# josehu07/summerset

Hardware: NVIDIA B200
Metric: RS shard GB/s on the fused RSPaxos accept step (RS(3,2) encode + quorum tally); consensus slots committed/s in slots_committed_per_s (higher is better)
Workload: dtype u8

## Files before the change

summerset_b200/csrc/horner_row_kernels.cuh:

```cuda
#pragma once
#include "device_common.cuh"
#include "static_codes.hpp"

namespace ssb {

using dev::funnel16;
using dev::keep_bytes;
using dev::msb_mask;

#ifndef SS_KMAXP
#define SS_KMAXP 8
#endif

struct EncRowGen {
    const uint8_t *data;
    uint64_t data_stride;
    uint8_t *plane[16];
    uint64_t shard_stride;
    uint32_t emit_data;
    dev::FlagWait wait;
    uint32_t n, len, L, vpc, fast_cols;
    uint32_t d, p;
    uint32_t pack_m, tail_ctas, ntail;
    const uint32_t *hmT8;
    uint8_t top[SS_KMAXP];
    const uint64_t *planes;
    uint32_t R, threshold;
    uint64_t *committed;
    uint32_t *commit_bar;
};

__device__ __forceinline__ uint32_t xtime_word(uint32_t x) { return ((x * 2u) & 0xfefefefeu) ^ (msb_mask(x) & 0x1d1d1d1du); }

template <int D, bool MASKED, bool EXACT>
__device__ __forceinline__ int row_load_column(const EncRowGen &P, const uint8_t *__restrict__ src, uint32_t k, uint4 (&x)[D]) {
    auto clamp16 = [](int64_t r) { return r > 16 ? 16 : (r < 0 ? 0 : static_cast<int>(r)); };
    const int d = EXACT ? D : static_cast<int>(P.d);
    uint4 lo[D], hi[D];
#pragma unroll
    for (int i = 0; i < D; ++i) {
        lo[i] = make_uint4(0u, 0u, 0u, 0u);
        hi[i] = lo[i];
        if (i < d) {
            const uint32_t pos = static_cast<uint32_t>(i) * P.L + k;
            const uint32_t s = (static_cast<uint32_t>(i) * P.L) & 15u;
            const int nv = MASKED ? clamp16(static_cast<int64_t>(P.len) - pos) : 16;
            if (!MASKED || nv > 0) lo[i] = dev::ldg128(src + pos - s);
            if (s != 0u && (!MASKED || static_cast<int>(s) + nv > 16)) hi[i] = dev::ldg128(src + pos - s + 16u);
        }
    }
    const int onv = MASKED ? clamp16(static_cast<int64_t>(P.L) - k) : 16;
#pragma unroll
    for (int i = 0; i < D; ++i) {
        x[i] = lo[i];
        if (i < d) {
            const uint32_t s = (static_cast<uint32_t>(i) * P.L) & 15u;
            if (s != 0u) x[i] = funnel16(lo[i], hi[i], s);
            if (MASKED) {
                const int nv = clamp16(static_cast<int64_t>(P.len) - (static_cast<uint32_t>(i) * P.L + k));
                x[i] = keep_bytes(x[i], nv < onv ? nv : onv);
            }
        }
    }
    return onv;
}

template <int CODE, int J, int D>
__device__ __forceinline__ uint4 static_parity_row(const uint4 (&x)[D]) {
    static_assert(D == static_code_d(CODE), "static code width");
    constexpr int top = static_code_top(CODE, J);
    uint4 acc = make_uint4(0u, 0u, 0u, 0u);
#pragma unroll
    for (int kk = 7; kk >= 0; --kk) {
        if (kk > top) continue;
        if (kk != top) {
            acc.x = xtime_word(acc.x); acc.y = xtime_word(acc.y);
            acc.z = xtime_word(acc.z); acc.w = xtime_word(acc.w);
        }
#pragma unroll
        for (int i = 0; i < D; ++i)
            if ((static_code_coef(CODE, J, i) >> kk) & 1u) {
                acc.x ^= x[i].x; acc.y ^= x[i].y; acc.z ^= x[i].z; acc.w ^= x[i].w;
            }
    }
    return acc;
}

template <int D, int CODE, bool MASKED>
__device__ __forceinline__ void parity_rows(const EncRowGen &P, const uint4 (&x)[D], int onv, uint64_t out_off) {
    if (P.emit_data) {
#pragma unroll
        for (int i = 0; i < D; ++i)
            if (CODE != kCodeGeneric || static_cast<uint32_t>(i) < P.d) dev::stg128_cs(P.plane[i] + out_off, x[i]);
    }
    if constexpr (CODE != kCodeGeneric) {
        static_assert(D == static_code_d(CODE), "static code width");
#pragma unroll
        for (int j = 0; j < static_code_p(CODE); ++j) {
            const int top = static_code_top(CODE, j);
            uint4 acc = make_uint4(0u, 0u, 0u, 0u);
#pragma unroll
            for (int kk = 7; kk >= 0; --kk) {
                if (kk > top) continue;
                if (kk != top) {
                    acc.x = xtime_word(acc.x); acc.y = xtime_word(acc.y);
                    acc.z = xtime_word(acc.z); acc.w = xtime_word(acc.w);
                }
#pragma unroll
                for (int i = 0; i < D; ++i)
                    if ((static_code_coef(CODE, j, i) >> kk) & 1u) {
                        acc.x ^= x[i].x; acc.y ^= x[i].y; acc.z ^= x[i].z; acc.w ^= x[i].w;
                    }
            }
            if (MASKED) acc = keep_bytes(acc, onv);
            dev::stg128_cs(P.plane[D + j] + out_off, acc);
        }
    } else {
        for (uint32_t j = 0; j < P.p; ++j) {
            const uint4 *hm = reinterpret_cast<const uint4 *>(P.hmT8 + j * 64u);
            uint4 acc = make_uint4(0u, 0u, 0u, 0u);
            const int top = P.top[j];
            for (int kk = top; kk >= 0; --kk) {
                const uint4 m0 = __ldg(hm + kk * 2);
                const uint4 m1 = D > 4 ? __ldg(hm + kk * 2 + 1) : make_uint4(0u, 0u, 0u, 0u);
                const uint32_t mk[8] = {m0.x, m0.y, m0.z, m0.w, m1.x, m1.y, m1.z, m1.w};
                if (kk != top) {
                    acc.x = xtime_word(acc.x); acc.y = xtime_word(acc.y);
                    acc.z = xtime_word(acc.z); acc.w = xtime_word(acc.w);
                }
#pragma unroll
                for (int i = 0; i < D; ++i) {
                    acc.x ^= x[i].x & mk[i];
                    acc.y ^= x[i].y & mk[i];
                    acc.z ^= x[i].z & mk[i];
                    acc.w ^= x[i].w & mk[i];
                }
            }
            if (MASKED) acc = keep_bytes(acc, onv);
            dev::stg128_cs(P.plane[P.d + j] + out_off, acc);
        }
    }
}

template <int D, int CODE, bool MASKED>
__device__ __forceinline__ void horner_row_column(const EncRowGen &P, const uint8_t *__restrict__ src, uint64_t out_off, uint32_t k) {
    uint4 x[D];
    const int onv = row_load_column<D, MASKED, CODE != kCodeGeneric>(P, src, k, x);
    parity_rows<D, CODE, MASKED>(P, x, onv, out_off + k);
}

template <int D, bool ALIGNED>
struct RawColumn {
    uint4 lo[D];
    uint4 hi[ALIGNED ? 1 : D];
};
template <int D, bool ALIGNED, bool EXACT>
__device__ __forceinline__ void raw_issue(const EncRowGen &P, const uint8_t *__restrict__ src, uint32_t k, RawColumn<D, ALIGNED> &r) {
    const int d = EXACT ? D : static_cast<int>(P.d);
#pragma unroll
    for (int i = 0; i < D; ++i) {
        if (i < d) {
            const uint32_t pos = static_cast<uint32_t>(i) * P.L + k;
            const uint32_t s = ALIGNED ? 0u : (static_cast<uint32_t>(i) * P.L) & 15u;
            r.lo[i] = dev::ldg128(src + pos - s);
            if constexpr (!ALIGNED) {
                if (i > 0) {
                    r.hi[i] = make_uint4(0u, 0u, 0u, 0u);
                    if (s != 0u) r.hi[i] = dev::ldg128(src + pos - s + 16u);
                }
            }
        } else {
            r.lo[i] = make_uint4(0u, 0u, 0u, 0u);
        }
    }
}
template <int D, bool ALIGNED, bool EXACT>
__device__ __forceinline__ void raw_finish(const EncRowGen &P, const RawColumn<D, ALIGNED> &r, uint4 (&x)[D]) {
    const int d = EXACT ? D : static_cast<int>(P.d);
#pragma unroll
    for (int i = 0; i < D; ++i) {
        x[i] = r.lo[i];
        if constexpr (!ALIGNED) {
            if (i > 0 && i < d) {
                const uint32_t s = (static_cast<uint32_t>(i) * P.L) & 15u;
                if (s != 0u) x[i] = funnel16(r.lo[i], r.hi[i], s);
            }
        }
    }
}

template <int D, int CODE, int MAXT, int MINB>
__global__ void __launch_bounds__(MAXT, MINB) horner_encode_row_kernel(const __grid_constant__ EncRowGen P) {
    const uint32_t lane = threadIdx.x & 31u, wid = threadIdx.x >> 5, nblk = blockDim.x >> 5;
    if (P.emit_data) dev::cta_wait_flags(P.wait);
    if (P.planes != nullptr) {
        const uint32_t per = (P.n + gridDim.x - 1) / gridDim.x;
        const uint32_t lo = blockIdx.x * per;
        const uint32_t hi = lo + per < P.n ? lo + per : P.n;
        for (uint32_t g = lo + threadIdx.x; g < hi; g += blockDim.x) {
            const uint64_t w = dev::tally_word(P.planes, P.R, P.n, g, P.threshold);
            P.committed[g] = w;
            if (P.commit_bar != nullptr) P.commit_bar[g] = dev::commit_prefix(w);
        }
    }
    uint32_t wb = wid;
#pragma unroll 1
    for (uint32_t g = blockIdx.x; g < P.n; g += gridDim.x) {
        const uint8_t *src = P.data + static_cast<uint64_t>(g) * P.data_stride;
        const uint64_t out_off = static_cast<uint64_t>(g) * P.shard_stride;
        for (uint32_t vb = 0; vb < P.vpc; vb += blockDim.x) {
            const uint32_t v = vb + wb * 32u + lane;
            const bool masked = vb + wb * 32u + 32u > P.fast_cols;
            if (v >= P.vpc) continue;
            if (!masked) horner_row_column<D, CODE, false>(P, src, out_off, v * 16u);
            else horner_row_column<D, CODE, true>(P, src, out_off, v * 16u);
        }
        wb = (wb + 1u == nblk) ? 0u : wb + 1u;
    }
}

template <int D, bool ALIGNED, bool PIPE>
SSB_HD constexpr int packed_min_blocks() {
    if (!PIPE) return D <= 3 ? 6 : D <= 5 ? 5 : D <= 6 ? 4 : 3;
    constexpr int need = 4 * D + (ALIGNED ? 4 * D : 8 * D - 4) + 22;
    constexpr int b = 65536 / (256 * need);
    return b > 6 ? 6 : (b < 1 ? 1 : b);
}

template <int D, int CODE, bool ALIGNED, bool PIPE>
__global__ void __launch_bounds__(256, packed_min_blocks<D, ALIGNED, PIPE>()) horner_encode_packed_kernel(const __grid_constant__ EncRowGen P) {
    if (P.emit_data) dev::cta_wait_flags(P.wait);
    if (P.planes != nullptr) {
        const uint32_t per = (P.n + gridDim.x - 1) / gridDim.x;
        const uint32_t lo = blockIdx.x * per;
        const uint32_t hi = lo + per < P.n ? lo + per : P.n;
        for (uint32_t g = lo + threadIdx.x; g < hi; g += blockDim.x) {
            const uint64_t w = dev::tally_word(P.planes, P.R, P.n, g, P.threshold);
            P.committed[g] = w;
            if (P.commit_bar != nullptr) P.commit_bar[g] = dev::commit_prefix(w);
        }
    }
    if (blockIdx.x < P.tail_ctas) {
        const uint64_t item = static_cast<uint64_t>(blockIdx.x) * blockDim.x + threadIdx.x;
        const uint64_t g = P.ntail == 1u ? item : item / P.ntail;
        if (g >= P.n) return;
        const uint32_t col = P.fast_cols + static_cast<uint32_t>(item - g * P.ntail);
        horner_row_column<D, CODE, true>(P, P.data + g * P.data_stride, g * P.shard_stride, col * 16u);
        return;
    }
    const uint32_t cg = threadIdx.x / P.fast_cols;
    const uint32_t k = (threadIdx.x - cg * P.fast_cols) * 16u;
    if (cg >= P.pack_m) return;
    const uint64_t step = static_cast<uint64_t>(gridDim.x - P.tail_ctas) * P.pack_m;
    uint64_t g = static_cast<uint64_t>(blockIdx.x - P.tail_ctas) * P.pack_m + cg;
    if (g >= P.n) return;
    if constexpr (!PIPE) {
#pragma unroll 1
        for (; g < P.n; g += step)
            horner_row_column<D, CODE, false>(P, P.data + g * P.data_stride, g * P.shard_stride, k);
        return;
    }
    RawColumn<D, ALIGNED> raw;
    raw_issue<D, ALIGNED, CODE != kCodeGeneric>(P, P.data + g * P.data_stride, k, raw);
#pragma unroll 1
    while (true) {
        uint4 x[D];
        raw_finish<D, ALIGNED, CODE != kCodeGeneric>(P, raw, x);
        const uint64_t gn = g + step;
        if (gn < P.n) raw_issue<D, ALIGNED, CODE != kCodeGeneric>(P, P.data + gn * P.data_stride, k, raw);
        parity_rows<D, CODE, false>(P, x, 16, g * P.shard_stride + k);
        if (gn >= P.n) break;
        g = gn;
    }
}


}
```

summerset_b200/csrc/jit.cu:

```cuda
#include <dlfcn.h>
#include <nvrtc.h>

#include <cstdio>
#include <cstring>
#include <mutex>
#include <string>
#include <vector>

#include "gf256.hpp"
#include "ss_internal.hpp"
#include "static_codes.hpp"

namespace ssb {

static const char *kJitSource =
#include "jit_source.inc"
    ;

struct NvrtcApi {
    void *handle = nullptr;
    nvrtcResult (*CreateProgram)(nvrtcProgram *, const char *, const char *, int, const char *const *, const char *const *) = nullptr;
    nvrtcResult (*DestroyProgram)(nvrtcProgram *) = nullptr;
    nvrtcResult (*CompileProgram)(nvrtcProgram, int, const char *const *) = nullptr;
    nvrtcResult (*AddNameExpression)(nvrtcProgram, const char *) = nullptr;
    nvrtcResult (*GetLoweredName)(nvrtcProgram, const char *, const char **) = nullptr;
    nvrtcResult (*GetCUBINSize)(nvrtcProgram, size_t *) = nullptr;
    nvrtcResult (*GetCUBIN)(nvrtcProgram, char *) = nullptr;
    nvrtcResult (*GetProgramLogSize)(nvrtcProgram, size_t *) = nullptr;
    nvrtcResult (*GetProgramLog)(nvrtcProgram, char *) = nullptr;
    const char *(*GetErrorString)(nvrtcResult) = nullptr;
    bool ok = false;
};

static NvrtcApi &nvrtc_api() {
    static NvrtcApi api;
    static std::once_flag once;
    std::call_once(once, [] {
        const char *names[] = {"libnvrtc.so.12", "libnvrtc.so", "/usr/local/cuda/lib64/libnvrtc.so.12", "/usr/local/cuda/lib64/libnvrtc.so"};
        for (const char *n : names) {
            api.handle = dlopen(n, RTLD_NOW | RTLD_LOCAL);
            if (api.handle) break;
        }
        if (!api.handle) return;
#define SS_NVRTC_SYM(field, sym) *reinterpret_cast<void **>(&api.field) = dlsym(api.handle, sym)
        SS_NVRTC_SYM(CreateProgram, "nvrtcCreateProgram");
        SS_NVRTC_SYM(DestroyProgram, "nvrtcDestroyProgram");
        SS_NVRTC_SYM(CompileProgram, "nvrtcCompileProgram");
        SS_NVRTC_SYM(AddNameExpression, "nvrtcAddNameExpression");
        SS_NVRTC_SYM(GetLoweredName, "nvrtcGetLoweredName");
        SS_NVRTC_SYM(GetCUBINSize, "nvrtcGetCUBINSize");
        SS_NVRTC_SYM(GetCUBIN, "nvrtcGetCUBIN");
        SS_NVRTC_SYM(GetProgramLogSize, "nvrtcGetProgramLogSize");
        SS_NVRTC_SYM(GetProgramLog, "nvrtcGetProgramLog");
        SS_NVRTC_SYM(GetErrorString, "nvrtcGetErrorString");
#undef SS_NVRTC_SYM
        api.ok = api.CreateProgram && api.DestroyProgram && api.CompileProgram && api.AddNameExpression && api.GetLoweredName &&
                 api.GetCUBINSize && api.GetCUBIN && api.GetProgramLogSize && api.GetProgramLog && api.GetErrorString;
    });
    return api;
}

static int row_min_blocks(int d) { return d <= 4 ? 12 : d == 5 ? 10 : d == 6 ? 8 : 6; }

int jit_compile(int d, int p, const uint8_t *rows, int which, std::vector<char> &cubin, std::string &name, std::string &log) {
    NvrtcApi &rt = nvrtc_api();
    if (!rt.ok) { log = "libnvrtc could not be loaded"; return SS_ERR_UNSUPPORTED; }
    if (d < 1 || d > 8 || p < 1 || p > 8 || which < 0 || which > 4) { log = "run-time specialisation covers d <= 8, p <= 8"; return SS_ERR_UNSUPPORTED; }
    std::string coefs;
    char tmp[16];
    for (int i = 0; i < d * p; ++i) {
        snprintf(tmp, sizeof tmp, "%s0x%02xu", i ? "," : "", rows[i]);
        coefs += tmp;
    }
    const std::string def_d = "-DSS_JIT_D=" + std::to_string(d), def_p = "-DSS_JIT_P=" + std::to_string(p), def_c = "-DSS_JIT_COEFS=" + coefs;
    const char *opts[] = {"--gpu-architecture=sm_100a", "-std=c++17", def_d.c_str(), def_p.c_str(), def_c.c_str()};
    nvrtcProgram prog = nullptr;
    nvrtcResult r = rt.CreateProgram(&prog, kJitSource, "summerset_b200_jit.cu", 0, nullptr, nullptr);
    if (r != NVRTC_SUCCESS) { log = std::string("nvrtcCreateProgram: ") + rt.GetErrorString(r); return SS_ERR_UNSUPPORTED; }
    const std::string D = std::to_string(d);
    const std::string exprs[5] = {
        "&ssb::horner_encode_row_kernel<" + D + ", ssb::kCodeJit, 128, " + std::to_string(row_min_blocks(d)) + ">",
        "&ssb::horner_encode_row_kernel<" + D + ", ssb::kCodeJit, 256, 3>",
        "&ssb::horner_encode_packed_kernel<" + D + ", ssb::kCodeJit, true, true>",
        "&ssb::horner_encode_packed_kernel<" + D + ", ssb::kCodeJit, false, true>",
        "&ssb::horner_encode_packed_kernel<" + D + ", ssb::kCodeJit, false, false>"};
    rt.AddNameExpression(prog, exprs[which].c_str());
    r = rt.CompileProgram(prog, 5, opts);
    size_t ls = 0;
    rt.GetProgramLogSize(prog, &ls);
    if (ls > 1) { log.resize(ls); rt.GetProgramLog(prog, &log[0]); }
    if (r != NVRTC_SUCCESS) {
        log = std::string("nvrtcCompileProgram: ") + rt.GetErrorString(r) + "\n" + log;
        rt.DestroyProgram(&prog);
        return SS_ERR_UNSUPPORTED;
    }
    const char *low = nullptr;
    if (rt.GetLoweredName(prog, exprs[which].c_str(), &low) != NVRTC_SUCCESS || low == nullptr) {
        log = "nvrtcGetLoweredName failed for " + exprs[which];
        rt.DestroyProgram(&prog);
        return SS_ERR_UNSUPPORTED;
    }
    name = low;
    size_t cs = 0;
    rt.GetCUBINSize(prog, &cs);
    cubin.resize(cs);
    r = rt.GetCUBIN(prog, cubin.data());
    rt.DestroyProgram(&prog);
    if (r != NVRTC_SUCCESS || cs == 0) { log = "nvrtcGetCUBIN failed"; return SS_ERR_UNSUPPORTED; }
    return SS_OK;
}

int jit_ensure(ss_rs_coder *c, int which) {
    if (c->jit_state[which] > 0) return SS_OK;
    if (c->jit_state[which] < 0) return SS_ERR_UNSUPPORTED;
    c->jit_state[which] = -1;
    std::vector<char> cubin;
    std::string name, log;
    const uint8_t *rows = c->matrix.data() + size_t(c->d) * c->d;
    if (jit_compile(c->d, c->p, rows, which, cubin, name, log) != SS_OK) { c->jit_message = log; return SS_ERR_UNSUPPORTED; }
    cudaLibrary_t lib = nullptr;
    cudaError_t e = cudaLibraryLoadData(&lib, cubin.data(), nullptr, nullptr, 0, nullptr, nullptr, 0);
    if (e != cudaSuccess) {
        cudaGetLastError();
        c->jit_message = std::string("cudaLibraryLoadData: ") + cudaGetErrorString(e);
        return SS_ERR_UNSUPPORTED;
    }
    cudaKernel_t k = nullptr;
    e = cudaLibraryGetKernel(&k, lib, name.c_str());
    if (e != cudaSuccess) {
        cudaGetLastError();
        cudaLibraryUnload(lib);
        c->jit_message = std::string("cudaLibraryGetKernel(") + name + "): " + cudaGetErrorString(e);
        return SS_ERR_UNSUPPORTED;
    }
    c->jit_kernel[which] = k;
    c->jit_library[which] = lib;
    c->jit_state[which] = 1;
    c->jit_message = "specialised by NVRTC (" + name + ", " + std::to_string(cubin.size()) + " bytes of sm_100a code)";
    return SS_OK;
}

void jit_release(ss_rs_coder *c) {
    for (int i = 0; i < 5; ++i) {
        if (c->jit_library[i]) cudaLibraryUnload(static_cast<cudaLibrary_t>(c->jit_library[i]));
        c->jit_library[i] = nullptr;
        c->jit_state[i] = 0;
    }
}

}

extern "C" {

long ss_jit_selftest(int d, int p, char *log, size_t log_cap) {
    if (log && log_cap) log[0] = 0;
    ssb::gf::Matrix M;
    try {
        M = ssb::gf::coding_matrix(d, p);
    } catch (const std::exception &ex) {
        if (log && log_cap) snprintf(log, log_cap, "%s", ex.what());
        return SS_ERR_INVALID_ARG;
    }
    long total = 0;
    for (int which = 0; which < 5; ++which) {
        std::vector<char> cubin;
        std::string name, msg;
        const int rc = ssb::jit_compile(d, p, M.v.data() + size_t(d) * d, which, cubin, name, msg);
        if (rc != SS_OK) {
            if (log && log_cap) snprintf(log, log_cap, "%s", msg.c_str());
            return rc;
        }
        total += static_cast<long>(cubin.size());
    }
    return total;
}

const char *ss_rs_jit_status(const ss_rs_coder *c) {
    if (c == nullptr) return "null coder";
    if (c->static_code >= 0 || c->is_rs32) return "compile-time code table (no run-time specialisation needed)";
    if (c->jit_message.empty()) return "not specialised yet (happens on the first batched encode)";
    return c->jit_message.c_str();
}

}
```

summerset_b200/csrc/rs_kernels.cu:

```cuda
#include <cstring>

#include "device_common.cuh"
#include "ss_internal.hpp"
#include "static_codes.hpp"
#include "rs32_decode.cuh"
#include "horner_row_kernels.cuh"

namespace ssb {

using dev::funnel16;
using dev::keep_bytes;
using dev::load16;
using dev::msb_mask;
using dev::store16;
using dev::xtime4;

constexpr int kThreads = 256;


__device__ __forceinline__ void rs32_word(uint32_t a, uint32_t b, uint32_t c, uint32_t &p0,
                                          uint32_t &p1) {
    const uint32_t t = a ^ b;
    const uint32_t u = a ^ c;
    p0 = t ^ c;
// ... 1206 lines not shown
            Rw.fast_cols = len >= 2u * L ? lim / 16u : 0u;
            Rw.s1 = L & 15u; Rw.s2 = (2u * L) & 15u;
            Rw.emit_data = ((g.flags & SS_RS_EMIT_DATA) || g.plane_ptrs != nullptr) ? 1u : 0u;
            Rw.planes = nullptr; Rw.R = 0; Rw.threshold = 0; Rw.committed = nullptr; Rw.commit_bar = nullptr;
            if (tally != nullptr && tally->planes != nullptr) {
                Rw.planes = tally->planes; Rw.R = tally->R; Rw.threshold = tally->threshold;
                Rw.committed = tally->committed; Rw.commit_bar = tally->commit_bar;
            }
            Rw.wait = g.wait;
            const uint32_t threads = vpc > 256u ? 256u : ((vpc + 31u) & ~31u);
            if (vpc > 256u) {
                const uint64_t items = g.n * ((vpc + 255u) / 256u);
                uint64_t ctas = static_cast<uint64_t>(ctx->sm_count) * 8ull * 16ull;
                if (ctas > items) ctas = items;
                Rw.chunk = 0; Rw.st_mode = static_cast<uint32_t>((coder->variant >> 8) & 3); Rw.rotate = 0;
                if (Rw.emit_data) rs32_encode_row_kernel<true, 256, 4, true><<<static_cast<uint32_t>(ctas), 256, 0, st>>>(Rw);
                else rs32_encode_row_kernel<false, 256, 4, true><<<static_cast<uint32_t>(ctas), 256, 0, st>>>(Rw);
                coder->last_kernel = Rw.planes ? "rs32_encode_row_kernel<segmented>+tally" : "rs32_encode_row_kernel<segmented>";
                SS_CUDA(cudaGetLastError());
                ctx->launches++;
                return SS_OK;
            }
            uint32_t per_sm = 2048u / threads; if (per_sm > 32u) per_sm = 32u;
            const int vr = coder->variant & 15, vchunk = (coder->variant >> 4) & 1, vw = (coder->variant >> 5) & 7;
            static const uint64_t kWaves[8] = {64, 1, 32, 4, 16, 256, 128, 8};
            const uint64_t waves = kWaves[vw];
            uint64_t ctas = static_cast<uint64_t>(ctx->sm_count) * per_sm * waves;
            if (ctas > g.n) ctas = g.n;
            Rw.chunk = 0;
            Rw.st_mode = static_cast<uint32_t>((coder->variant >> 8) & 3);
            Rw.rotate = ((coder->variant >> 10) & 1) ? 0u : 1u;
            if (vchunk) { Rw.chunk = static_cast<uint32_t>((g.n + ctas - 1) / ctas); ctas = (g.n + Rw.chunk - 1) / Rw.chunk; }
            const uint32_t grid = static_cast<uint32_t>(ctas);
            if (threads > 128) {
                if (Rw.emit_data) rs32_encode_row_kernel<true, 256, 4><<<grid, threads, 0, st>>>(Rw);
                else rs32_encode_row_kernel<false, 256, 4><<<grid, threads, 0, st>>>(Rw);
            } else if (Rw.emit_data) rs32_encode_row_kernel<true, 128, 8><<<grid, threads, 0, st>>>(Rw);
            else if (vr == 3) rs32_encode_row_kernel<false, 128, 16><<<grid, threads, 0, st>>>(Rw);
            else if (vr == 6) rs32_encode_row_kernel<false, 128, 8><<<grid, threads, 0, st>>>(Rw);
            else if (vr == 7) rs32_encode_row_kernel<false, 128, 9><<<grid, threads, 0, st>>>(Rw);
            else rs32_encode_row_kernel<false, 128, 12><<<grid, threads, 0, st>>>(Rw);
            coder->last_kernel = Rw.planes ? "rs32_encode_row_kernel+tally" : "rs32_encode_row_kernel";
            SS_CUDA(cudaGetLastError());
            ctx->launches++;
            return SS_OK;
        }

        if (!use_rs32 && d <= 8 && coder->enc_hmT8 != nullptr && (coder->variant & 15) != 5 && (coder->variant & 15) != 1 &&
            padded && vpc >= 1 && g.n <= 0xffffffffull &&
            ((reinterpret_cast<uintptr_t>(g.data) | g.data_stride) & 15u) == 0u &&
            (tally == nullptr || tally->planes == nullptr || tally->G == g.n)) {
            EncRowGen Rg;
            Rg.data = g.data; Rg.data_stride = g.data_stride;
            for (int j = 0; j < 16; ++j) {
                if (j >= d + p) Rg.plane[j] = nullptr;
                else if (g.plane_ptrs != nullptr) Rg.plane[j] = g.plane_ptrs[j];
                else Rg.plane[j] = g.parity + (static_cast<int64_t>(j) - d) * static_cast<int64_t>(g.plane_stride);
            }
            Rg.emit_data = ((g.flags & SS_RS_EMIT_DATA) || g.plane_ptrs != nullptr) ? 1u : 0u;
            Rg.wait = g.wait;
            Rg.shard_stride = g.shard_stride; Rg.n = static_cast<uint32_t>(g.n); Rg.len = len; Rg.L = L; Rg.vpc = vpc;
            const uint64_t last_shard_bytes = static_cast<uint64_t>(len) >= static_cast<uint64_t>(d - 1) * L
                                                  ? static_cast<uint64_t>(len) - static_cast<uint64_t>(d - 1) * L : 0;
            Rg.fast_cols = static_cast<uint32_t>((last_shard_bytes < L ? last_shard_bytes : L) / 16u);
            Rg.d = static_cast<uint32_t>(d); Rg.p = static_cast<uint32_t>(p);
            Rg.hmT8 = static_cast<const uint32_t *>(coder->enc_hmT8);
            for (int j = 0; j < kMaxP; ++j) Rg.top[j] = coder->enc_top[j];
            Rg.planes = nullptr; Rg.R = 0; Rg.threshold = 0; Rg.committed = nullptr; Rg.commit_bar = nullptr;
            if (tally != nullptr && tally->planes != nullptr) {
                Rg.planes = tally->planes; Rg.R = tally->R; Rg.threshold = tally->threshold;
                Rg.committed = tally->committed; Rg.commit_bar = tally->commit_bar;
            }
            int sc = ((coder->variant >> 11) & 1) ? kCodeGeneric : coder->static_code;
            const bool jit_allowed = sc == kCodeGeneric && !((coder->variant >> 11) & 1) && !((coder->variant >> 17) & 1);
            auto launch_jit = [&](int which, uint32_t grid_x, uint32_t block_x) -> int {
                void *args[] = {&Rg};
                SS_CUDA(cudaLaunchKernel(reinterpret_cast<const void *>(coder->jit_kernel[which]), dim3(grid_x), dim3(block_x), args, 0, st));
                return SS_OK;
            };
            const uint32_t fc = Rg.fast_cols;
            const uint32_t row_threads = vpc > 256u ? 256u : ((vpc + 31u) & ~31u);
            bool packed = (fc != vpc || row_threads != vpc) && vpc <= 256u;
            if ((coder->variant >> 13) & 1) packed = false;
            if ((coder->variant >> 14) & 1) packed = true;
            const bool pipe = (L & 15u) == 0u || ((coder->variant >> 15) & 1);
            if (jit_allowed) {
                const int which = packed ? ((L & 15u) == 0u ? 2 : pipe ? 3 : 4) : (row_threads > 128u ? 1 : 0);
                if (jit_ensure(coder, which) == SS_OK) sc = kCodeJit;
            }
            if (packed) {
                uint32_t T = 256, m = fc ? 256u / fc : 0u;
                if (fc) {
                    double best = -1.0;
                    for (uint32_t t = 256; t >= 64; t -= 32) {
                        const uint32_t mm = t / fc;
                        const double eff = static_cast<double>(mm * fc) / t;
                        if (eff > best + 1e-9) { best = eff; T = t; m = mm; }
                    }
                }
                Rg.pack_m = m;
                Rg.ntail = vpc - fc;
                const uint64_t tail_items = g.n * Rg.ntail;
                const uint64_t tail_ctas = (tail_items + T - 1) / T;
                uint64_t main_ctas = 0;
                if (m) {
                    const uint32_t dcap = d <= 2 ? 2 : d == 3 ? 3 : d == 4 ? 4 : d <= 6 ? 6 : 8;
                    const uint32_t dt = sc != kCodeGeneric ? static_cast<uint32_t>(d) : dcap;
                    const uint32_t reg_need = 4u * dt + ((L & 15u) == 0u ? 4u * dt : 8u * dt - 4u) + 22u;
                    uint32_t rb = 65536u / (256u * reg_need); rb = rb > 6u ? 6u : (rb < 1u ? 1u : rb);
                    if (!pipe) rb = dt <= 3 ? 6u : dt <= 5 ? 5u : dt <= 6 ? 4u : 3u;
                    const uint32_t resident_threads = 256u * rb;
                    main_ctas = static_cast<uint64_t>(ctx->sm_count) * (resident_threads / T) * 64ull;
                    const uint64_t need = (g.n + m - 1) / m;
                    if (main_ctas > need) main_ctas = need;
                }
                if (tail_ctas + main_ctas <= 0x7fffffffull) {
                    Rg.tail_ctas = static_cast<uint32_t>(tail_ctas);
                    const uint32_t grid = static_cast<uint32_t>(tail_ctas + main_ctas);
                    auto gop = [&](auto DC, auto CC) {
                        constexpr int kD = decltype(DC)::value, kC = decltype(CC)::value;
                        if ((L & 15u) == 0u) horner_encode_packed_kernel<kD, kC, true, true><<<grid, T, 0, st>>>(Rg);
                        else if (pipe) horner_encode_packed_kernel<kD, kC, false, true><<<grid, T, 0, st>>>(Rg);
                        else horner_encode_packed_kernel<kD, kC, false, false><<<grid, T, 0, st>>>(Rg);
                    };
                    auto gop_static = [&](auto CC) {
                        constexpr int C = decltype(CC)::value;
                        gop(std::integral_constant<int, static_code_d(C)>{}, CC);
                    };
                    switch (sc) {
                        case kCodeJit: SS_TRY(launch_jit((L & 15u) == 0u ? 2 : pipe ? 3 : 4, grid, T)); break;
                        case kCode21: gop_static(std::integral_constant<int, kCode21>{}); break;
                        case kCode43: gop_static(std::integral_constant<int, kCode43>{}); break;
                        case kCode54: gop_static(std::integral_constant<int, kCode54>{}); break;
                        case kCode42: gop_static(std::integral_constant<int, kCode42>{}); break;
                        case kCode31: gop_static(std::integral_constant<int, kCode31>{}); break;
                        default:
                            SS_TRY(dispatch_d(d, [&](auto DC) {
                                gop(DC, std::integral_constant<int, kCodeGeneric>{});
                                return SS_OK;
                            }));
                    }
                    if (sc == kCodeJit)
                        coder->last_kernel = Rg.planes ? "horner_encode_packed_kernel<nvrtc>+tally" : "horner_encode_packed_kernel<nvrtc>";
                    else if (sc != kCodeGeneric)
                        coder->last_kernel = Rg.planes ? "horner_encode_packed_kernel<static code>+tally" : "horner_encode_packed_kernel<static code>";
                    else
                        coder->last_kernel = Rg.planes ? "horner_encode_packed_kernel+tally" : "horner_encode_packed_kernel";
                    SS_CUDA(cudaGetLastError());
                    ctx->launches++;
                    return SS_OK;
                }
            }
            Rg.pack_m = 0; Rg.tail_ctas = 0; Rg.ntail = 0;
            const uint32_t threads = row_threads;
            if (sc == kCodeJit && jit_ensure(coder, threads > 128u ? 1 : 0) != SS_OK) sc = kCodeGeneric;
            uint32_t per_sm = 2048u / threads; if (per_sm > 32u) per_sm = 32u;
            uint64_t ctas = static_cast<uint64_t>(ctx->sm_count) * per_sm * 64ull;
            if (ctas > g.n) ctas = g.n;
            const uint32_t grid = static_cast<uint32_t>(ctas);
            const int vbits = coder->variant & 15;
            auto go = [&](auto DC, auto CC) {
                constexpr int kD = decltype(DC)::value, kC = decltype(CC)::value;
                const int vdef = kD <= 4 ? 0 : kD == 5 ? 2 : kD == 6 ? 3 : 4;
                const int vb = (vbits >= 2 && vbits <= 4) ? vbits : vdef;
                if (threads > 128) horner_encode_row_kernel<kD, kC, 256, 3><<<grid, threads, 0, st>>>(Rg);
                else if (vb == 2) horner_encode_row_kernel<kD, kC, 128, 10><<<grid, threads, 0, st>>>(Rg);
                else if (vb == 3) horner_encode_row_kernel<kD, kC, 128, 8><<<grid, threads, 0, st>>>(Rg);
                else if (vb == 4) horner_encode_row_kernel<kD, kC, 128, 6><<<grid, threads, 0, st>>>(Rg);
                else horner_encode_row_kernel<kD, kC, 128, 12><<<grid, threads, 0, st>>>(Rg);
            };
            auto go_static = [&](auto CC) {
                constexpr int C = decltype(CC)::value;
                go(std::integral_constant<int, static_code_d(C)>{}, CC);
            };
            switch (sc) {
                case kCodeJit: SS_TRY(launch_jit(threads > 128 ? 1 : 0, grid, threads)); break;
                case kCode21: go_static(std::integral_constant<int, kCode21>{}); break;
                case kCode43: go_static(std::integral_constant<int, kCode43>{}); break;
                case kCode54: go_static(std::integral_constant<int, kCode54>{}); break;
                case kCode42: go_static(std::integral_constant<int, kCode42>{}); break;
                case kCode31: go_static(std::integral_constant<int, kCode31>{}); break;
                default:
                    SS_TRY(dispatch_d(d, [&](auto DC) {
                        go(DC, std::integral_constant<int, kCodeGeneric>{});
                        return SS_OK;
                    }));
            }
            if (sc == kCodeJit)
                coder->last_kernel = Rg.planes ? "horner_encode_row_kernel<nvrtc>+tally" : "horner_encode_row_kernel<nvrtc>";
            else if (sc != kCodeGeneric)
                coder->last_kernel = Rg.planes ? "horner_encode_row_kernel<static code>+tally" : "horner_encode_row_kernel<static code>";
            else
                coder->last_kernel = Rg.planes ? "horner_encode_row_kernel+tally" : "horner_encode_row_kernel";
            SS_CUDA(cudaGetLastError());
            ctx->launches++;
            return SS_OK;
        }
        const uint64_t max_cw = vpc ? (0xffffff00ull / vpc) : g.n;
        uint64_t done = 0;
        bool tally_pending = tally != nullptr && tally->planes != nullptr;
        do {
            const uint64_t nc = (g.n - done) < max_cw ? (g.n - done) : max_cw;
            EncUniform E;
            E.data = g.data + done * g.data_stride;
            E.data_stride = g.data_stride;
            E.len = len; E.L = L; E.vpc = vpc;
            E.parity = g.parity + done * g.shard_stride;
            E.plane_stride = g.plane_stride; E.shard_stride = g.shard_stride;
            E.n = nc;
            E.total = static_cast<uint32_t>(nc * vpc);
            E.padded = (padded ? 1u : 0u) | ((g.flags & SS_RS_EMIT_DATA) ? 2u : 0u);
            E.planes = nullptr; E.R = 0; E.threshold = 0; E.G = 0; E.committed = nullptr; E.commit_bar = nullptr;
            uint64_t threads = E.total;
            if (tally_pending) {
                if (tally->G > 0xffffff00ull) return set_error(SS_ERR_INVALID_ARG, "too many groups for one fused launch");
                E.planes = tally->planes; E.R = tally->R; E.threshold = tally->threshold; E.G = tally->G;
                E.committed = tally->committed; E.commit_bar = tally->commit_bar;
                if (threads < tally->G) threads = tally->G;
                tally_pending = false;
            }
            if (threads == 0) break;
            const uint32_t grid = static_cast<uint32_t>((threads + kThreads - 1) / kThreads);
            if (use_rs32) {
                rs32_encode_uniform_kernel<<<grid, kThreads, 0, st>>>(E);
                coder->last_kernel = E.planes ? "rs32_encode_uniform_kernel+tally" : "rs32_encode_uniform_kernel";
            } else if (d <= 8 && (coder->variant & 15) != 5) {
                const uint32_t *prog = static_cast<const uint32_t *>(coder->enc_prog);
                SS_TRY(dispatch_d(d, [&](auto DC) {
                    horner_encode_uniform_kernel<decltype(DC)::value><<<grid, kThreads, 0, st>>>(E, prog, d, p);
                    return SS_OK;
                }));
                coder->last_kernel = "horner_encode_uniform_kernel";
            } else {
                const uint32_t *prog = static_cast<const uint32_t *>(coder->enc_prog);
                SS_TRY(dispatch_p(p, [&](auto PC) {
                    generic_encode_uniform_kernel<decltype(PC)::value><<<grid, kThreads, 0, st>>>(E, prog, d, p);
// ... 152 lines not shown
```

summerset_b200/csrc/ss_internal.hpp:

```cpp
#pragma once
#include <cuda_runtime.h>

#include <atomic>
#include <cstdint>
#include <cstdio>
#include <string>
#include <vector>

#include "../../include/summerset_b200.h"
#include "device_common.cuh"

namespace ssb {

int set_error(int code, const char *fmt, ...);
int cuda_error(cudaError_t e, const char *what, const char *file, int line);

#define SS_CUDA(call)                                                        \
    do {                                                                     \
        cudaError_t _e = (call);                                             \
        if (_e != cudaSuccess) return ::ssb::cuda_error(_e, #call, __FILE__, __LINE__); \
    } while (0)

#define SS_TRY(call)                \
    do {                            \
        int _rc = (call);           \
        if (_rc != SS_OK) return _rc; \
    } while (0)

constexpr int kMaxD = 32;
constexpr int kMaxP = 8;
struct ProgHeader {
    uint8_t n_out;
    uint8_t n_missing_data;
    uint8_t valid;
    uint8_t pad0;
    uint8_t src[kMaxD];
    uint8_t dst[kMaxP];
    uint8_t top[kMaxP];
    uint8_t topT[2];
    uint8_t chain1;
    uint8_t pad1[9];
};
static_assert(sizeof(ProgHeader) == 64, "ProgHeader must be 64 bytes");

struct FastProgHeader {
    uint8_t valid, n_out, chain1, pad0;
    uint8_t src[4];
    uint8_t dst[kMaxP];
    uint8_t top[kMaxP];
    uint8_t pad1[8];
};
static_assert(sizeof(FastProgHeader) == 32, "FastProgHeader must be 32 bytes");

}

struct ss_ctx {
    int device = -1;
    cudaStream_t stream = nullptr;
    bool owns_stream = false;
    int sm_count = 0;
    uint64_t launches = 0;
    std::atomic<int> live_handles{1};
    std::atomic<bool> closing{false};
    void *scratch = nullptr;
    size_t scratch_bytes = 0;
    static constexpr int kStages = 3;
    cudaStream_t h2d_stream = nullptr, d2h_stream = nullptr;
    cudaEvent_t ev_h2d[kStages] = {}, ev_kernel[kStages] = {}, ev_done[kStages] = {};
    bool pipeline_ready = false;
    void *stage_in[kStages] = {};
    void *stage_out[kStages] = {};
    size_t stage_in_bytes = 0, stage_out_bytes = 0;
    void *pinned = nullptr;
    size_t pinned_bytes = 0;
    uint32_t *dev_status = nullptr;
};

struct ss_rs_coder {
    ss_ctx *ctx = nullptr;
    int d = 0, p = 0;
    std::vector<uint8_t> matrix;
    bool is_rs32 = false;
    int variant = 0;
    const char *last_kernel = "none";
    void *enc_prog = nullptr;
    void *enc_hmT8 = nullptr;
    uint8_t enc_top[ssb::kMaxP] = {};
    int static_code = -1;
    void *dec_progs = nullptr;
    void *dec_progs_data = nullptr;
    void *fast_progs = nullptr;
    void *fast_progs_data = nullptr;
    size_t fast_stride = 0;
    size_t prog_stride = 0;
    bool batch_ok = false;
    bool dec_ok = false;
    int jit_state[5] = {};
    std::string jit_message;
    void *jit_library[5] = {};
    cudaKernel_t jit_kernel[5] = {};
    std::vector<uint8_t> verify_buf;
    std::vector<uint8_t *> verify_ptrs;
};

namespace ssb {

int ctx_bind(ss_ctx *ctx);
void ctx_retain(ss_ctx *ctx);
void ctx_release(ss_ctx *ctx);
int ctx_scratch(ss_ctx *ctx, size_t bytes, void **out);

struct EncGeom {
    const uint8_t *data;
    const uint64_t *data_off;
    const uint32_t *data_len;
    uint64_t data_stride;
    uint32_t uni_len;
    uint8_t *parity;
    uint64_t plane_stride;
    const uint64_t *par_off;
    uint64_t shard_stride;
    uint64_t n;
    uint32_t flags;
    uint8_t *const *plane_ptrs = nullptr;
    dev::FlagWait wait = {nullptr, 0, 0, 0, nullptr};
};

struct TallyArgs {
    const uint64_t *planes = nullptr;
    uint32_t R = 0, threshold = 0;
    uint64_t G = 0;
    uint64_t *committed = nullptr;
    uint32_t *commit_bar = nullptr;
};

int launch_rs_encode(ss_rs_coder *coder, const EncGeom &g, const TallyArgs *tally);
int match_static_code(int d, int p, const uint8_t *matrix);
int launch_rs_reconstruct(ss_rs_coder *coder, uint8_t *shards, uint64_t plane_stride,
                          const uint64_t *off, const uint32_t *data_len, const uint32_t *present,
                          uint64_t n, int data_only, int32_t *status, uint32_t flags);
int launch_rs_reconstruct_uniform(ss_rs_coder *coder, uint8_t *shards, uint64_t plane_stride, uint64_t shard_stride,
                                  uint32_t data_len, const uint32_t *present, uint64_t n, int data_only, int32_t *status);
int launch_tally_planes(ss_ctx *ctx, const uint64_t *planes, uint32_t R, uint64_t G, uint32_t thr,
                        uint64_t *committed, uint32_t *commit_bar);
int launch_tally_masks(ss_ctx *ctx, const void *masks, uint32_t mask_bytes, uint64_t n, uint32_t thr,
                       uint64_t *commit_bits);
int launch_ack_ingest(ss_ctx *ctx, const uint32_t *rec_group, const uint8_t *rec_slot,
                      const uint8_t *rec_peer, const uint64_t *rec_ballot, uint64_t n_records,
                      const uint64_t *bal_prepared, const uint64_t *inst_bal, const uint64_t *accepting,
                      uint32_t R, uint64_t G, uint64_t *planes);
int launch_tally_crossword(ss_ctx *ctx, const void *masks, uint32_t mask_bytes, const uint8_t *policy_idx,
                           uint64_t n, const uint32_t *policies_host, uint32_t n_policies,
                           uint32_t n_replicas, uint32_t T, uint32_t d, uint32_t majority, uint32_t f,
                           int balanced, uint64_t *commit_bits);
int launch_raft_scan(ss_ctx *ctx, const uint32_t *match, uint32_t n_peers, uint64_t G,
                     const uint32_t *last_commit, const uint32_t *log_end, const uint32_t *curr_term,
                     const uint32_t *terms, uint32_t window, uint32_t threshold, uint32_t *new_commit,
                     uint32_t *window_overflow, uint32_t ring = 0);
int launch_raft_scan_ring(ss_ctx *ctx, const uint32_t *match, uint32_t n_peers, uint64_t G, const uint32_t *last_commit,
                          const uint32_t *log_end, const uint32_t *curr_term, const uint32_t *terms, uint32_t window,
                          uint32_t threshold, uint32_t *new_commit);
int launch_crossword_lut(ss_ctx *ctx, const uint32_t *d_policies, uint32_t n_policies, uint32_t n_replicas, uint32_t T, uint32_t d,
                         uint32_t majority, uint32_t f, int balanced, uint32_t *d_lut_bits);

int jit_ensure(ss_rs_coder *coder, int which);
void jit_release(ss_rs_coder *coder);

int make_flag_wait(ss_ctx *ctx, const ss_step_sync *sync, dev::FlagWait *out);
int launch_flag_signal(ss_ctx *ctx, const ss_step_sync *sync);
int launch_flag_wait(ss_ctx *ctx, const dev::FlagWait &w);
int launch_follower_ack(ss_ctx *ctx, const uint64_t *ack_src, uint64_t *const *ack_dst, uint32_t R, uint64_t G,
                        const dev::FlagWait &wait);

int launch_kth_match(ss_ctx *ctx, const uint32_t *match, uint32_t n_peers, uint64_t G, uint32_t k, uint32_t *out);
int launch_prepare_merge(ss_ctx *ctx, const uint64_t *vote_bal, const uint32_t *vote_mask, uint32_t R, uint64_t N,
                         const uint8_t *acks_cnt, uint32_t d, uint32_t population, uint32_t f, uint64_t *max_bal,
                         uint32_t *merged, uint8_t *action);

int launch_crossword_distribute(ss_rs_coder *coder, const uint8_t *data, const uint64_t *data_off,
                                const uint32_t *data_len, const uint8_t *spr, const uint64_t *rep_off, uint64_t n,
                                uint8_t *const *replica_logs, uint32_t n_replicas);

int launch_frame_accept(ss_ctx *ctx, const uint8_t *plane, uint64_t shard_stride, uint32_t shard_idx, uint32_t d, uint32_t p,
// ... 9 lines not shown
```

Baseline: 6655.

## Restructure packed encode kernel into warp-strided codeword groups with fused Horner step

Replaces the packed encode kernel's tail-CTA split and the software-pipelined raw load path with one scheme. A fixed group of 32 codewords is mapped across warps: fast columns are located with a magic-number divide and masked tail columns are handled one codeword per lane, which removes the separate tail CTAs and the host-side thread-count search. For static codes the Horner doubling step is fused into a mulhi/mad sequence that XORs in the next term. The cost is the loss of the explicit load prefetch pipeline and the aligned/unaligned specialisations, and the JIT variants drop from five to three.

```diff
diff --git a/summerset_b200/csrc/horner_row_kernels.cuh b/summerset_b200/csrc/horner_row_kernels.cuh
--- a/summerset_b200/csrc/horner_row_kernels.cuh
+++ b/summerset_b200/csrc/horner_row_kernels.cuh
@@ -21,7 +21,7 @@
     dev::FlagWait wait;
     uint32_t n, len, L, vpc, fast_cols;
     uint32_t d, p;
-    uint32_t pack_m, tail_ctas, ntail;
+    uint32_t fc_magic;
     const uint32_t *hmT8;
     uint8_t top[SS_KMAXP];
     const uint64_t *planes;
@@ -31,6 +31,14 @@
 };
 
 __device__ __forceinline__ uint32_t xtime_word(uint32_t x) { return ((x * 2u) & 0xfefefefeu) ^ (msb_mask(x) & 0x1d1d1d1du); }
+
+__device__ __forceinline__ uint32_t horner_step_word(uint32_t acc, uint32_t u) {
+    const uint32_t t = acc & 0x80808080u;
+    const uint32_t red = __umulhi(t, 0x1du << 25);
+    uint32_t sh;
+    asm("mad.lo.u32 %0, %1, 0xfffffffe, %2;" : "=r"(sh) : "r"(t), "r"(acc * 2u));
+    return sh ^ red ^ u;
+}
 
 template <int D, bool MASKED, bool EXACT>
 __device__ __forceinline__ int row_load_column(const EncRowGen &P, const uint8_t *__restrict__ src, uint32_t k, uint4 (&x)[D]) {
@@ -86,7 +94,31 @@
     return acc;
 }
 
-template <int D, int CODE, bool MASKED>
+template <int CODE, int D>
+__device__ __forceinline__ uint4 static_parity_row_fma(int j, const uint4 (&x)[D]) {
+    static_assert(D == static_code_d(CODE), "static code width");
+    const int top = static_code_top(CODE, j);
+    uint4 acc = make_uint4(0u, 0u, 0u, 0u);
+#pragma unroll
+    for (int kk = 7; kk >= 0; --kk) {
+        if (kk > top) continue;
+        uint4 u = make_uint4(0u, 0u, 0u, 0u);
+#pragma unroll
+        for (int i = 0; i < D; ++i)
+            if ((static_code_coef(CODE, j, i) >> kk) & 1u) {
+                u.x ^= x[i].x; u.y ^= x[i].y; u.z ^= x[i].z; u.w ^= x[i].w;
+            }
+        if (kk == top) {
+            acc = u;
+        } else {
+            acc.x = horner_step_word(acc.x, u.x); acc.y = horner_step_word(acc.y, u.y);
+            acc.z = horner_step_word(acc.z, u.z); acc.w = horner_step_word(acc.w, u.w);
+        }
+    }
+    return acc;
+}
+
+template <int D, int CODE, bool MASKED, bool FMA_STEP = false>
 __device__ __forceinline__ void parity_rows(const EncRowGen &P, const uint4 (&x)[D], int onv, uint64_t out_off) {
     if (P.emit_data) {
 #pragma unroll
@@ -97,6 +129,12 @@
         static_assert(D == static_code_d(CODE), "static code width");
 #pragma unroll
         for (int j = 0; j < static_code_p(CODE); ++j) {
+            if constexpr (FMA_STEP) {
+                uint4 acc = static_parity_row_fma<CODE, D>(j, x);
+                if (MASKED) acc = keep_bytes(acc, onv);
+                dev::stg128_cs(P.plane[D + j] + out_off, acc);
+                continue;
+            }
             const int top = static_code_top(CODE, j);
             uint4 acc = make_uint4(0u, 0u, 0u, 0u);
 #pragma unroll
@@ -142,51 +180,11 @@
     }
 }
 
-template <int D, int CODE, bool MASKED>
+template <int D, int CODE, bool MASKED, bool FMA_STEP = false>
 __device__ __forceinline__ void horner_row_column(const EncRowGen &P, const uint8_t *__restrict__ src, uint64_t out_off, uint32_t k) {
     uint4 x[D];
     const int onv = row_load_column<D, MASKED, CODE != kCodeGeneric>(P, src, k, x);
-    parity_rows<D, CODE, MASKED>(P, x, onv, out_off + k);
-}
-
-template <int D, bool ALIGNED>
-struct RawColumn {
-    uint4 lo[D];
-    uint4 hi[ALIGNED ? 1 : D];
-};
-template <int D, bool ALIGNED, bool EXACT>
-__device__ __forceinline__ void raw_issue(const EncRowGen &P, const uint8_t *__restrict__ src, uint32_t k, RawColumn<D, ALIGNED> &r) {
-    const int d = EXACT ? D : static_cast<int>(P.d);
-#pragma unroll
-    for (int i = 0; i < D; ++i) {
-        if (i < d) {
-            const uint32_t pos = static_cast<uint32_t>(i) * P.L + k;
-            const uint32_t s = ALIGNED ? 0u : (static_cast<uint32_t>(i) * P.L) & 15u;
-            r.lo[i] = dev::ldg128(src + pos - s);
-            if constexpr (!ALIGNED) {
-                if (i > 0) {
-                    r.hi[i] = make_uint4(0u, 0u, 0u, 0u);
-                    if (s != 0u) r.hi[i] = dev::ldg128(src + pos - s + 16u);
-                }
-            }
-        } else {
-            r.lo[i] = make_uint4(0u, 0u, 0u, 0u);
-        }
-    }
-}
-template <int D, bool ALIGNED, bool EXACT>
-__device__ __forceinline__ void raw_finish(const EncRowGen &P, const RawColumn<D, ALIGNED> &r, uint4 (&x)[D]) {
-    const int d = EXACT ? D : static_cast<int>(P.d);
-#pragma unroll
-    for (int i = 0; i < D; ++i) {
-        x[i] = r.lo[i];
-        if constexpr (!ALIGNED) {
-            if (i > 0 && i < d) {
-                const uint32_t s = (static_cast<uint32_t>(i) * P.L) & 15u;
-                if (s != 0u) x[i] = funnel16(r.lo[i], r.hi[i], s);
-            }
-        }
-    }
+    parity_rows<D, CODE, MASKED, FMA_STEP>(P, x, onv, out_off + k);
 }
 
 template <int D, int CODE, int MAXT, int MINB>
@@ -219,16 +217,13 @@
     }
 }
 
-template <int D, bool ALIGNED, bool PIPE>
-SSB_HD constexpr int packed_min_blocks() {
-    if (!PIPE) return D <= 3 ? 6 : D <= 5 ? 5 : D <= 6 ? 4 : 3;
-    constexpr int need = 4 * D + (ALIGNED ? 4 * D : 8 * D - 4) + 22;
-    constexpr int b = 65536 / (256 * need);
-    return b > 6 ? 6 : (b < 1 ? 1 : b);
-}
-
-template <int D, int CODE, bool ALIGNED, bool PIPE>
-__global__ void __launch_bounds__(256, packed_min_blocks<D, ALIGNED, PIPE>()) horner_encode_packed_kernel(const __grid_constant__ EncRowGen P) {
+constexpr uint32_t kPackCodewords = 32;
+
+template <int D>
+SSB_HD constexpr int packed_min_blocks() { return D <= 2 ? 6 : D <= 4 ? 5 : D <= 6 ? 4 : 3; }
+
+template <int D, int CODE>
+__global__ void __launch_bounds__(256, packed_min_blocks<D>()) horner_encode_packed_kernel(const __grid_constant__ EncRowGen P) {
     if (P.emit_data) dev::cta_wait_flags(P.wait);
     if (P.planes != nullptr) {
         const uint32_t per = (P.n + gridDim.x - 1) / gridDim.x;
@@ -240,39 +235,27 @@
             if (P.commit_bar != nullptr) P.commit_bar[g] = dev::commit_prefix(w);
         }
     }
-    if (blockIdx.x < P.tail_ctas) {
-        const uint64_t item = static_cast<uint64_t>(blockIdx.x) * blockDim.x + threadIdx.x;
-        const uint64_t g = P.ntail == 1u ? item : item / P.ntail;
-        if (g >= P.n) return;
-        const uint32_t col = P.fast_cols + static_cast<uint32_t>(item - g * P.ntail);
-        horner_row_column<D, CODE, true>(P, P.data + g * P.data_stride, g * P.shard_stride, col * 16u);
-        return;
-    }
-    const uint32_t cg = threadIdx.x / P.fast_cols;
-    const uint32_t k = (threadIdx.x - cg * P.fast_cols) * 16u;
-    if (cg >= P.pack_m) return;
-    const uint64_t step = static_cast<uint64_t>(gridDim.x - P.tail_ctas) * P.pack_m;
-    uint64_t g = static_cast<uint64_t>(blockIdx.x - P.tail_ctas) * P.pack_m + cg;
-    if (g >= P.n) return;
-    if constexpr (!PIPE) {
+    constexpr bool kFma = CODE != kCodeGeneric;
+    const uint32_t lane = threadIdx.x & 31u, nwarps = blockDim.x >> 5;
+    const uint64_t step = static_cast<uint64_t>(gridDim.x) * kPackCodewords;
+    uint64_t base = static_cast<uint64_t>(blockIdx.x) * kPackCodewords;
+    uint32_t w = threadIdx.x >> 5;
+    while (w >= P.vpc) { w -= P.vpc; base += step; }
 #pragma unroll 1
-        for (; g < P.n; g += step)
-            horner_row_column<D, CODE, false>(P, P.data + g * P.data_stride, g * P.shard_stride, k);
-        return;
-    }
-    RawColumn<D, ALIGNED> raw;
-    raw_issue<D, ALIGNED, CODE != kCodeGeneric>(P, P.data + g * P.data_stride, k, raw);
-#pragma unroll 1
-    while (true) {
-        uint4 x[D];
-        raw_finish<D, ALIGNED, CODE != kCodeGeneric>(P, raw, x);
-        const uint64_t gn = g + step;
-        if (gn < P.n) raw_issue<D, ALIGNED, CODE != kCodeGeneric>(P, P.data + gn * P.data_stride, k, raw);
-        parity_rows<D, CODE, false>(P, x, 16, g * P.shard_stride + k);
-        if (gn >= P.n) break;
-        g = gn;
-    }
-}
-
-
-}
+    while (base < P.n) {
+        if (w < P.fast_cols) {
+            const uint32_t idx = w * 32u + lane;
+            const uint32_t cg = __umulhi(idx << 11, P.fc_magic);
+            const uint32_t k = (idx - cg * P.fast_cols) * 16u;
+            const uint64_t g = base + cg;
+            if (g < P.n) horner_row_column<D, CODE, false, kFma>(P, P.data + g * P.data_stride, g * P.shard_stride, k);
+        } else {
+            const uint64_t g = base + lane;
+            if (g < P.n) horner_row_column<D, CODE, true, kFma>(P, P.data + g * P.data_stride, g * P.shard_stride, w * 16u);
+        }
+        w += nwarps;
+        while (w >= P.vpc) { w -= P.vpc; base += step; }
+    }
+}
+
+}
diff --git a/summerset_b200/csrc/jit.cu b/summerset_b200/csrc/jit.cu
--- a/summerset_b200/csrc/jit.cu
+++ b/summerset_b200/csrc/jit.cu
@@ -65,7 +65,7 @@
 int jit_compile(int d, int p, const uint8_t *rows, int which, std::vector<char> &cubin, std::string &name, std::string &log) {
     NvrtcApi &rt = nvrtc_api();
     if (!rt.ok) { log = "libnvrtc could not be loaded"; return SS_ERR_UNSUPPORTED; }
-    if (d < 1 || d > 8 || p < 1 || p > 8 || which < 0 || which > 4) { log = "run-time specialisation covers d <= 8, p <= 8"; return SS_ERR_UNSUPPORTED; }
+    if (d < 1 || d > 8 || p < 1 || p > 8 || which < 0 || which >= kJitKernels) { log = "run-time specialisation covers d <= 8, p <= 8"; return SS_ERR_UNSUPPORTED; }
     std::string coefs;
     char tmp[16];
     for (int i = 0; i < d * p; ++i) {
@@ -78,12 +78,10 @@
     nvrtcResult r = rt.CreateProgram(&prog, kJitSource, "summerset_b200_jit.cu", 0, nullptr, nullptr);
     if (r != NVRTC_SUCCESS) { log = std::string("nvrtcCreateProgram: ") + rt.GetErrorString(r); return SS_ERR_UNSUPPORTED; }
     const std::string D = std::to_string(d);
-    const std::string exprs[5] = {
+    const std::string exprs[kJitKernels] = {
         "&ssb::horner_encode_row_kernel<" + D + ", ssb::kCodeJit, 128, " + std::to_string(row_min_blocks(d)) + ">",
         "&ssb::horner_encode_row_kernel<" + D + ", ssb::kCodeJit, 256, 3>",
-        "&ssb::horner_encode_packed_kernel<" + D + ", ssb::kCodeJit, true, true>",
-        "&ssb::horner_encode_packed_kernel<" + D + ", ssb::kCodeJit, false, true>",
-        "&ssb::horner_encode_packed_kernel<" + D + ", ssb::kCodeJit, false, false>"};
+        "&ssb::horner_encode_packed_kernel<" + D + ", ssb::kCodeJit>"};
     rt.AddNameExpression(prog, exprs[which].c_str());
     r = rt.CompileProgram(prog, 5, opts);
     size_t ls = 0;
@@ -141,7 +139,7 @@
 }
 
 void jit_release(ss_rs_coder *c) {
-    for (int i = 0; i < 5; ++i) {
+    for (int i = 0; i < kJitKernels; ++i) {
         if (c->jit_library[i]) cudaLibraryUnload(static_cast<cudaLibrary_t>(c->jit_library[i]));
         c->jit_library[i] = nullptr;
         c->jit_state[i] = 0;
@@ -162,7 +160,7 @@
         return SS_ERR_INVALID_ARG;
     }
     long total = 0;
-    for (int which = 0; which < 5; ++which) {
+    for (int which = 0; which < ssb::kJitKernels; ++which) {
         std::vector<char> cubin;
         std::string name, msg;
         const int rc = ssb::jit_compile(d, p, M.v.data() + size_t(d) * d, which, cubin, name, msg);
diff --git a/summerset_b200/csrc/rs_kernels.cu b/summerset_b200/csrc/rs_kernels.cu
--- a/summerset_b200/csrc/rs_kernels.cu
+++ b/summerset_b200/csrc/rs_kernels.cu
@@ -1312,76 +1312,53 @@
             const uint32_t row_threads = vpc > 256u ? 256u : ((vpc + 31u) & ~31u);
             bool packed = (fc != vpc || row_threads != vpc) && vpc <= 256u;
             if ((coder->variant >> 13) & 1) packed = false;
-            if ((coder->variant >> 14) & 1) packed = true;
-            const bool pipe = (L & 15u) == 0u || ((coder->variant >> 15) & 1);
+            if ((coder->variant >> 14) & 1) packed = vpc <= 256u;
             if (jit_allowed) {
-                const int which = packed ? ((L & 15u) == 0u ? 2 : pipe ? 3 : 4) : (row_threads > 128u ? 1 : 0);
+                const int which = packed ? 2 : (row_threads > 128u ? 1 : 0);
                 if (jit_ensure(coder, which) == SS_OK) sc = kCodeJit;
             }
             if (packed) {
-                uint32_t T = 256, m = fc ? 256u / fc : 0u;
-                if (fc) {
-                    double best = -1.0;
-                    for (uint32_t t = 256; t >= 64; t -= 32) {
-                        const uint32_t mm = t / fc;
-                        const double eff = static_cast<double>(mm * fc) / t;
-                        if (eff > best + 1e-9) { best = eff; T = t; m = mm; }
-                    }
+                Rg.fc_magic = fc ? ((1u << 21) + fc - 1u) / fc : 0u;
+                const uint32_t dt = sc != kCodeGeneric ? static_cast<uint32_t>(d)
+                                                       : d <= 2 ? 2 : d == 3 ? 3 : d == 4 ? 4 : d <= 6 ? 6 : 8;
+                const uint32_t rb = static_cast<uint32_t>(dt <= 2 ? packed_min_blocks<2>() : dt <= 4 ? packed_min_blocks<4>()
+                                                          : dt <= 6 ? packed_min_blocks<6>() : packed_min_blocks<8>());
+                const uint64_t passes = (g.n + kPackCodewords - 1) / kPackCodewords;
+                uint64_t ctas = static_cast<uint64_t>(ctx->sm_count) * rb * 16ull;
+                if (ctas > passes) ctas = passes;
+                const uint32_t grid = static_cast<uint32_t>(ctas);
+                auto gop = [&](auto DC, auto CC) {
+                    constexpr int kD = decltype(DC)::value, kC = decltype(CC)::value;
+                    horner_encode_packed_kernel<kD, kC><<<grid, 256, 0, st>>>(Rg);
+                };
+                auto gop_static = [&](auto CC) {
+                    constexpr int C = decltype(CC)::value;
+                    gop(std::integral_constant<int, static_code_d(C)>{}, CC);
+                };
+                switch (sc) {
+                    case kCodeJit: SS_TRY(launch_jit(2, grid, 256)); break;
+                    case kCode21: gop_static(std::integral_constant<int, kCode21>{}); break;
+                    case kCode43: gop_static(std::integral_constant<int, kCode43>{}); break;
+                    case kCode54: gop_static(std::integral_constant<int, kCode54>{}); break;
+                    case kCode42: gop_static(std::integral_constant<int, kCode42>{}); break;
+                    case kCode31: gop_static(std::integral_constant<int, kCode31>{}); break;
+                    default:
+                        SS_TRY(dispatch_d(d, [&](auto DC) {
+                            gop(DC, std::integral_constant<int, kCodeGeneric>{});
+                            return SS_OK;
+                        }));
                 }
-                Rg.pack_m = m;
-                Rg.ntail = vpc - fc;
-                const uint64_t tail_items = g.n * Rg.ntail;
-                const uint64_t tail_ctas = (tail_items + T - 1) / T;
-                uint64_t main_ctas = 0;
-                if (m) {
-                    const uint32_t dcap = d <= 2 ? 2 : d == 3 ? 3 : d == 4 ? 4 : d <= 6 ? 6 : 8;
-                    const uint32_t dt = sc != kCodeGeneric ? static_cast<uint32_t>(d) : dcap;
-                    const uint32_t reg_need = 4u * dt + ((L & 15u) == 0u ? 4u * dt : 8u * dt - 4u) + 22u;
-                    uint32_t rb = 65536u / (256u * reg_need); rb = rb > 6u ? 6u : (rb < 1u ? 1u : rb);
-                    if (!pipe) rb = dt <= 3 ? 6u : dt <= 5 ? 5u : dt <= 6 ? 4u : 3u;
-                    const uint32_t resident_threads = 256u * rb;
-                    main_ctas = static_cast<uint64_t>(ctx->sm_count) * (resident_threads / T) * 64ull;
-                    const uint64_t need = (g.n + m - 1) / m;
-                    if (main_ctas > need) main_ctas = need;
-                }
-                if (tail_ctas + main_ctas <= 0x7fffffffull) {
-                    Rg.tail_ctas = static_cast<uint32_t>(tail_ctas);
-                    const uint32_t grid = static_cast<uint32_t>(tail_ctas + main_ctas);
-                    auto gop = [&](auto DC, auto CC) {
-                        constexpr int kD = decltype(DC)::value, kC = decltype(CC)::value;
-                        if ((L & 15u) == 0u) horner_encode_packed_kernel<kD, kC, true, true><<<grid, T, 0, st>>>(Rg);
-                        else if (pipe) horner_encode_packed_kernel<kD, kC, false, true><<<grid, T, 0, st>>>(Rg);
-                        else horner_encode_packed_kernel<kD, kC, false, false><<<grid, T, 0, st>>>(Rg);
-                    };
-                    auto gop_static = [&](auto CC) {
-                        constexpr int C = decltype(CC)::value;
-                        gop(std::integral_constant<int, static_code_d(C)>{}, CC);
-                    };
-                    switch (sc) {
-                        case kCodeJit: SS_TRY(launch_jit((L & 15u) == 0u ? 2 : pipe ? 3 : 4, grid, T)); break;
-                        case kCode21: gop_static(std::integral_constant<int, kCode21>{}); break;
-                        case kCode43: gop_static(std::integral_constant<int, kCode43>{}); break;
-                        case kCode54: gop_static(std::integral_constant<int, kCode54>{}); break;
-                        case kCode42: gop_static(std::integral_constant<int, kCode42>{}); break;
-                        case kCode31: gop_static(std::integral_constant<int, kCode31>{}); break;
-                        default:
-                            SS_TRY(dispatch_d(d, [&](auto DC) {
-                                gop(DC, std::integral_constant<int, kCodeGeneric>{});
-                                return SS_OK;
-                            }));
-                    }
-                    if (sc == kCodeJit)
-                        coder->last_kernel = Rg.planes ? "horner_encode_packed_kernel<nvrtc>+tally" : "horner_encode_packed_kernel<nvrtc>";
-                    else if (sc != kCodeGeneric)
-                        coder->last_kernel = Rg.planes ? "horner_encode_packed_kernel<static code>+tally" : "horner_encode_packed_kernel<static code>";
-                    else
-                        coder->last_kernel = Rg.planes ? "horner_encode_packed_kernel+tally" : "horner_encode_packed_kernel";
-                    SS_CUDA(cudaGetLastError());
-                    ctx->launches++;
-                    return SS_OK;
-                }
-            }
-            Rg.pack_m = 0; Rg.tail_ctas = 0; Rg.ntail = 0;
+                if (sc == kCodeJit)
+                    coder->last_kernel = Rg.planes ? "horner_encode_packed_kernel<nvrtc>+tally" : "horner_encode_packed_kernel<nvrtc>";
+                else if (sc != kCodeGeneric)
+                    coder->last_kernel = Rg.planes ? "horner_encode_packed_kernel<static code>+tally" : "horner_encode_packed_kernel<static code>";
+                else
+                    coder->last_kernel = Rg.planes ? "horner_encode_packed_kernel+tally" : "horner_encode_packed_kernel";
+                SS_CUDA(cudaGetLastError());
+                ctx->launches++;
+                return SS_OK;
+            }
+            Rg.fc_magic = 0;
             const uint32_t threads = row_threads;
             if (sc == kCodeJit && jit_ensure(coder, threads > 128u ? 1 : 0) != SS_OK) sc = kCodeGeneric;
             uint32_t per_sm = 2048u / threads; if (per_sm > 32u) per_sm = 32u;
diff --git a/summerset_b200/csrc/ss_internal.hpp b/summerset_b200/csrc/ss_internal.hpp
--- a/summerset_b200/csrc/ss_internal.hpp
+++ b/summerset_b200/csrc/ss_internal.hpp
@@ -52,6 +52,8 @@
 };
 static_assert(sizeof(FastProgHeader) == 32, "FastProgHeader must be 32 bytes");
 
+constexpr int kJitKernels = 3;
+
 }
 
 struct ss_ctx {
@@ -95,10 +97,10 @@
     size_t prog_stride = 0;
     bool batch_ok = false;
     bool dec_ok = false;
-    int jit_state[5] = {};
+    int jit_state[ssb::kJitKernels] = {};
     std::string jit_message;
-    void *jit_library[5] = {};
-    cudaKernel_t jit_kernel[5] = {};
+    void *jit_library[ssb::kJitKernels] = {};
+    cudaKernel_t jit_kernel[ssb::kJitKernels] = {};
     std::vector<uint8_t> verify_buf;
     std::vector<uint8_t *> verify_ptrs;
 };
```

After: 6654 (median of 6 runs). About the same (-0.0%).
